# AlexeyAB/yolo2_light

Measured on NVIDIA H100. Metric: images/sec, higher is better.
Workload: dtype bf16

## Files before the change

yolo2_light_b200/csrc/yb_conv_tc.cu:

```cuda
#include <cuda.h>
#include <cuda_bf16.h>
#include <cuda_runtime.h>

#include <algorithm>
#include <climits>
#include <cstdlib>
#include <cstring>
#include <string>
#include <type_traits>
#include <vector>

#include "yb_conv_tc.cuh"

namespace yb {

namespace {

constexpr int TC_BM = 128;
constexpr int TC_EPI_WARPS = 8;
constexpr int TC_THREADS = 32 * TC_EPI_WARPS + 32;
constexpr int TC_PRODUCER_WARP = TC_EPI_WARPS;
constexpr int TC_ACC_BAR = 3;

struct TcParams {
// ... 765 lines not shown
                const int img = J / p.PR, oy = J - img * p.PR - p.row_off;
                valid[h] = img < p.N && oy >= 0 && oy < p.OH && ox < p.OW;
            }
            const int nslab = (min(BN, p.n - n0) + SW - 1) / SW;
            if constexpr (ST) {
                const long long c0 = clock64();
                mbar_wait(stg_ready(wg), stg_phase);
                const long long dt = clock64() - c0;
                if (w != w_first) w_ready += dt;
                else if (p.stats && warp == 0 && lane == 0) p.stats[blockIdx.x * 16 + 3] = (unsigned long long)dt;
            }
            else mbar_wait(stg_ready(wg), stg_phase);
            stg_phase ^= 1u;
#pragma unroll
            for (int s = 0; s < BN / SW; ++s) {
                if (s >= nslab) break;
                const uint32_t slab = buf + (uint32_t)s * TILE;
#pragma unroll
                for (int jj = 0; jj < SW / 8; ++jj) {
                    const int j = s * (SW / 8) + jj;
                    const float2 b = *reinterpret_cast<const float2 *>(bias_s + n0 + 8 * j + cq);
#pragma unroll
                    for (int e = 0; e < 4; ++e) {
                        const float a = d[4 * j + e] + ((e & 1) ? b.y : b.x);
                        d[4 * j + e] = leaky ? fmaxf(a, 0.1f * a) : a;
                    }
                }
                if (has_res) {
                    uint32_t u[SW / 8][2];
#pragma unroll
                    for (int jj = 0; jj < SW / 8; ++jj)
#pragma unroll
                        for (int h = 0; h < 2; ++h)
                            asm volatile("ld.shared.b32 %0, [%1];" : "=r"(u[jj][h]) : "r"(slab + slab_off(rl + 8 * h, jj)));
#pragma unroll
                    for (int jj = 0; jj < SW / 8; ++jj) {
                        const int j = s * (SW / 8) + jj;
#pragma unroll
                        for (int h = 0; h < 2; ++h) {
                            float a = d[4 * j + 2 * h] + __uint_as_float(u[jj][h] << 16);
                            float c = d[4 * j + 2 * h + 1] + __uint_as_float(u[jj][h] & 0xffff0000u);
                            if (leaky2) { a = fmaxf(a, 0.1f * a); c = fmaxf(c, 0.1f * c); }
                            d[4 * j + 2 * h] = a; d[4 * j + 2 * h + 1] = c;
                        }
                    }
                }
#pragma unroll
                for (int jj = 0; jj < SW / 8; ++jj) {
                    const int j = s * (SW / 8) + jj;
#pragma unroll
                    for (int h = 0; h < 2; ++h) {
                        const uint32_t o = valid[h] ? pack_bf16x2(d[4 * j + 2 * h], d[4 * j + 2 * h + 1]) : 0u;
                        asm volatile("st.shared.b32 [%0], %1;" ::"r"(slab + slab_off(rl + 8 * h, jj)), "r"(o));
                    }
                }
                asm volatile("fence.proxy.async.shared::cta;" ::: "memory");
                __syncwarp();
                if (lane == 0) mbar_arrive(stg_full(wg, s));
            }
        }
    };
    auto by_kk = [&](auto bn_c) {
        if (p.kk == 4) run(bn_c, std::integral_constant<int, 4>{});
        else if (p.kk == 2) run(bn_c, std::integral_constant<int, 2>{});
        else run(bn_c, std::integral_constant<int, 1>{});
    };
    if (p.BN == 256) by_kk(std::integral_constant<int, 256>{});
    else if (p.BN == 128) by_kk(std::integral_constant<int, 128>{});
    else if (p.BN == 64) by_kk(std::integral_constant<int, 64>{});
    else by_kk(std::integral_constant<int, 32>{});
    if (ST && p.stats && warp == 0 && lane == 0) { p.stats[blockIdx.x * 16 + 2] = (unsigned long long)w_full; p.stats[blockIdx.x * 16 + 6] = (unsigned long long)(clock64() - t_begin);
                                                    p.stats[blockIdx.x * 16 + 8] = (unsigned long long)w_ready; }
}

struct StemTcP {
    const float *in;
    const unsigned char *in8;
    char *out; int out_ldc;
    const __nv_bfloat16 *w;
    const float *bias;
    int N, H, W, OHp, OWp, nf, act;
    long npix;
    int ntiles;
};

template <bool U8>
__global__ void __launch_bounds__(128) k_stem_tc(StemTcP p) {
    __shared__ __align__(1024) uint8_t a_tile[128 * 64];
    __shared__ __align__(1024) uint8_t b_tile[32 * 64];
    __shared__ __align__(16) float acc_s[128 * 36];
    __shared__ float bias_s[32];
    __shared__ unsigned long long optr[128];
    __shared__ float lut[U8 ? 256 : 1];
    const int t = threadIdx.x;
    if constexpr (U8) { lut[t] = (float)((double)(float)t / 255.0); lut[t + 128] = (float)((double)(float)(t + 128) / 255.0); }
    const uint32_t a_addr = smem_u32(a_tile), b_addr = smem_u32(b_tile), acc_addr = smem_u32(acc_s);
    if (t < 32) bias_s[t] = (t < p.nf) ? p.bias[t] : 0.f;
    {
        const int f = t >> 2, j = t & 3;
        const uint4 v = *reinterpret_cast<const uint4 *>(p.w + f * 32 + j * 8);
        *reinterpret_cast<uint4 *>(b_tile + f * 64 + ((j ^ ((f >> 1) & 3)) << 4)) = v;
    }
    __syncthreads();
    const uint32_t hi = ((8u * 64u) >> 4) | (2u << 30);
    const size_t plane = (size_t)p.H * p.W;
    for (int tile = blockIdx.x; tile < p.ntiles; tile += gridDim.x) {
        const unsigned pix = (unsigned)tile * 128u + (unsigned)t;
        const bool ok = pix < (unsigned)p.npix;
        int x = 0, y = 0, n = 0;
        if (ok) { const unsigned row = pix / (unsigned)p.W; x = (int)(pix - row * (unsigned)p.W); n = (int)(row / (unsigned)p.H); y = (int)(row - (unsigned)n * (unsigned)p.H); }
        uint32_t packed[16];
        {
            float v[32];
            if constexpr (U8) {
                const unsigned char *img8 = p.in8 + (size_t)n * 3 * plane;
                if (ok && x >= 1 && x + 1 < p.W && y >= 1 && y + 1 < p.H) {
                    const unsigned char *r1 = img8 + ((size_t)y * p.W + x) * 3, *r0 = r1 - (size_t)p.W * 3, *r2 = r1 + (size_t)p.W * 3;
#pragma unroll
                    for (int j = 0; j < 9; ++j) {
                        v[0 * 9 + j] = lut[__ldg(r0 - 3 + j)];
                        v[1 * 9 + j] = lut[__ldg(r1 - 3 + j)];
                        v[2 * 9 + j] = lut[__ldg(r2 - 3 + j)];
                    }
                } else {
#pragma unroll
                    for (int ky = 0; ky < 3; ++ky)
#pragma unroll
                        for (int kx = 0; kx < 3; ++kx) {
                            const int iy = y + ky - 1, ix = x + kx - 1;
                            const bool in_img = ok && iy >= 0 && iy < p.H && ix >= 0 && ix < p.W;
#pragma unroll
                            for (int c = 0; c < 3; ++c)
                                v[(ky * 3 + kx) * 3 + c] = in_img ? lut[__ldg(img8 + ((size_t)iy * p.W + ix) * 3 + c)] : 0.f;
                        }
                }
            } else {
            const float *img = p.in + (size_t)n * 3 * plane;
            if (ok && x >= 1 && x + 1 < p.W && y >= 1 && y + 1 < p.H) {
                const float *c0 = img + (size_t)y * p.W + x;
#pragma unroll
                for (int c = 0; c < 3; ++c) {
                    const float *r1 = c0 + (size_t)c * plane, *r0 = r1 - p.W, *r2 = r1 + p.W;
                    v[(0 * 3 + 0) * 3 + c] = __ldg(r0 - 1); v[(0 * 3 + 1) * 3 + c] = __ldg(r0); v[(0 * 3 + 2) * 3 + c] = __ldg(r0 + 1);
                    v[(1 * 3 + 0) * 3 + c] = __ldg(r1 - 1); v[(1 * 3 + 1) * 3 + c] = __ldg(r1); v[(1 * 3 + 2) * 3 + c] = __ldg(r1 + 1);
                    v[(2 * 3 + 0) * 3 + c] = __ldg(r2 - 1); v[(2 * 3 + 1) * 3 + c] = __ldg(r2); v[(2 * 3 + 2) * 3 + c] = __ldg(r2 + 1);
                }
            } else {
#pragma unroll
            for (int ky = 0; ky < 3; ++ky)
#pragma unroll
                for (int kx = 0; kx < 3; ++kx) {
                    const int iy = y + ky - 1, ix = x + kx - 1;
                    const bool in_img = ok && iy >= 0 && iy < p.H && ix >= 0 && ix < p.W;
#pragma unroll
                    for (int c = 0; c < 3; ++c)
                        v[(ky * 3 + kx) * 3 + c] = in_img ? __ldg(img + (size_t)c * plane + (size_t)iy * p.W + ix) : 0.f;
                }
            }
            }
#pragma unroll
            for (int k = 27; k < 32; ++k) v[k] = 0.f;
#pragma unroll
            for (int k = 0; k < 16; ++k) packed[k] = pack_bf16x2(v[2 * k], v[2 * k + 1]);
        }
#pragma unroll
        for (int j = 0; j < 4; ++j)
            *reinterpret_cast<uint4 *>(a_tile + t * 64 + ((j ^ ((t >> 1) & 3)) << 4)) =
                make_uint4(packed[4 * j], packed[4 * j + 1], packed[4 * j + 2], packed[4 * j + 3]);
        asm volatile("fence.proxy.async.shared::cta;" ::: "memory");
        __syncthreads();
        {
            float d0[16], d1[16];
#pragma unroll
            for (int i = 0; i < 16; ++i) { d0[i] = 0.f; d1[i] = 0.f; }
            wg_fence();
#pragma unroll
            for (int k = 0; k < 2; ++k) {
                const uint64_t bdesc = wg_desc(b_addr + 32u * k, hi);
                Wg<0, 32>::mma(d0, wg_desc(a_addr + 32u * k, hi), bdesc, (uint32_t)k);
                Wg<0, 32>::mma(d1, wg_desc(a_addr + 64u * 64u + 32u * k, hi), bdesc, (uint32_t)k);
            }
            wg_commit();
            wg_wait<0>();
            acc_store_frag(acc_addr, 36, 0, d0);
            acc_store_frag(acc_addr, 36, 64, d1);
        }
        __syncthreads();
        uint32_t acc[32];
        acc_ld32(acc_addr + 4u * 36u * (uint32_t)t, acc);
        char *orow = ok ? p.out + ((size_t)(n * p.OHp + y + 1) * p.OWp + x + 1) * (size_t)p.out_ldc * 2 : nullptr;
        if (p.nf == 32) {
            uint4 o[4];
#pragma unroll
            for (int g = 0; g < 4; ++g) {
                float r[8];
#pragma unroll
                for (int j = 0; j < 8; ++j) {
                    const float a = __uint_as_float(acc[g * 8 + j]) + bias_s[g * 8 + j];
                    r[j] = (p.act == ACT_LEAKY) ? fmaxf(a, 0.1f * a) : a;
                }
                o[g] = make_uint4(pack_bf16x2(r[0], r[1]), pack_bf16x2(r[2], r[3]), pack_bf16x2(r[4], r[5]), pack_bf16x2(r[6], r[7]));
            }
#pragma unroll
            for (int g = 0; g < 4; ++g) *reinterpret_cast<uint4 *>(a_tile + t * 64 + ((g ^ ((t >> 1) & 3)) << 4)) = o[g];
            optr[t] = (unsigned long long)(uintptr_t)orow;
            __syncthreads();
#pragma unroll
            for (int k = 0; k < 4; ++k) {
                const int j = t + 128 * k, px = j >> 2, part = j & 3;
                const unsigned long long dst = optr[px];
                if (dst)
                    *reinterpret_cast<uint4 *>(dst + (unsigned long long)(part * 16)) =
                        *reinterpret_cast<const uint4 *>(a_tile + px * 64 + ((part ^ ((px >> 1) & 3)) << 4));
            }
        } else if (ok) {
#pragma unroll
            for (int g = 0; g < 4; ++g) {
                if (g * 8 >= p.nf) break;
                float r[8];
#pragma unroll
                for (int j = 0; j < 8; ++j) {
                    const float a = __uint_as_float(acc[g * 8 + j]) + bias_s[g * 8 + j];
                    r[j] = (p.act == ACT_LEAKY) ? fmaxf(a, 0.1f * a) : a;
                }
                reinterpret_cast<uint4 *>(orow)[g] = make_uint4(pack_bf16x2(r[0], r[1]), pack_bf16x2(r[2], r[3]),
                                                                pack_bf16x2(r[4], r[5]), pack_bf16x2(r[6], r[7]));
            }
        }
        __syncthreads();
    }
}

typedef CUresult (*EncodeTiledFn)(CUtensorMap *, CUtensorMapDataType, cuuint32_t, void *, const cuuint64_t *,
                                  const cuuint64_t *, const cuuint32_t *, const cuuint32_t *, CUtensorMapInterleave,
                                  CUtensorMapSwizzle, CUtensorMapL2promotion, CUtensorMapFloatOOBfill);

EncodeTiledFn encode_fn() {
    static EncodeTiledFn fn = nullptr;
    if (!fn) {
        void *p = nullptr;
        cudaDriverEntryPointQueryResult q;
        if (cudaGetDriverEntryPoint("cuTensorMapEncodeTiled", &p, cudaEnableDefault, &q) != cudaSuccess || !p)
            fatal_throw("cuTensorMapEncodeTiled not available from the driver");
        fn = reinterpret_cast<EncodeTiledFn>(p);
    }
    return fn;
}

struct TcPlan {
    CUtensorMap tmA, tmB, tmO, tmO1, tmR;
    TcParams p;
    int grid;
    int threads;
    size_t smem;
    int pdl;
    char desc[96];
};

int pick_bk(int C) { return (C % 64 == 0) ? 64 : (C % 32 == 0) ? 32 : (C % 16 == 0) ? 16 : 0; }
int pick_bk_i8(int cpad) { return (cpad % 128 == 0) ? 128 : (cpad % 64 == 0) ? 64 : (cpad % 32 == 0) ? 32 : 0; }
int pick_bk_f32(int C) { return (C % 32 == 0) ? 32 : (C % 16 == 0) ? 16 : (C % 8 == 0) ? 8 : 0; }
int pick_bn(int n) { return n <= 32 ? 32 : n <= 64 ? 64 : 128; }
int pick_bn_reg(int n, long m_tiles, int kblocks, int sms) {
    int cap = 32;
    while (cap < n && cap < 256) cap *= 2;
    if (const char *e = getenv("YB_TC_BN")) {
        int bn = 32;
        while (bn * 2 <= std::min(atoi(e), cap)) bn *= 2;
        return bn;
    }
    int best = 32; double best_cost = 1e300;
    for (int bn = 32; bn <= cap; bn *= 2) {
        const long items = m_tiles * ((n + bn - 1) / bn);
        const double cost = (double)((items + sms - 1) / sms) * ((double)kblocks * (bn + 64) + 2.0 * bn);
        if (cost < best_cost) { best_cost = cost; best = bn; }
    }
    return best;
}

int grid_cap(int sms) {
    const char *e = getenv("YB_TC_GRID");
    return (e && atoi(e) > 0) ? std::min(sms, atoi(e)) : sms;
}

}

int tc_conv_supported(const Layer &l, const TV &in, const TV &out, bool out_bf16) {
    if (!out.base || (reinterpret_cast<uintptr_t>(out.base) & 15) != 0) return 0;
    if (out_bf16 ? (out.ldc % 8 != 0) : (out.ldc % 4 != 0)) return 0;
    if (l.activation != YB_LEAKY && l.activation != YB_LINEAR) return 0;
    if (pick_bk(l.c) == 0) return 0;
    if (in.ldc % 8 != 0 || (reinterpret_cast<uintptr_t>(in.base) & 15) != 0 || in.P != 1) return 0;
    const bool s1 = l.stride == 1 && ((l.size == 3 && l.pad == 1) || (l.size == 1 && l.pad == 0));
    const bool s2 = l.stride == 2 && l.size == 3 && l.pad == 1 && (l.h % 2 == 0) && (l.w % 2 == 0);
    if (!s1 && !s2) return 0;
    if (out_bf16 && l.n % 8 != 0) return 0;
    if (l.n < 8) return 0;
    return 1;
}

static void *make_plan_common(int kind, const Layer &l, const TV &in, const TV &out, bool out_bf16, const TV &res,
                              bool res_bf16, int act2, const void *d_weights_bf16, int ldn, const float *d_bias,
                              float alpha1, int *acc_out, int wide_rows = 0, int want_pool_tile = 0) {
    TcPlan *plan = new TcPlan();
    memset(plan, 0, sizeof(*plan));
    TcParams &p = plan->p;
    const bool i8 = kind == 1 || kind == 2;
    const int esz = kind == 3 ? 4 : i8 ? 1 : 2;
    const int cin = i8 ? in.ldc : l.c;
    const int BK = kind == 3 ? pick_bk_f32(l.c) : i8 ? pick_bk_i8(cin) : pick_bk(l.c);
    const bool reg = kind == 0 && out_bf16;
    p.kind = kind; p.alpha1 = alpha1; p.acc_out = acc_out;
// ... 141 lines not shown
    plan->threads = reg ? TCR_THREADS : TC_THREADS;
    if (getenv("YB_TC_STATS")) {
        cudaMalloc(&p.stats, sizeof(unsigned long long) * 16 * plan->grid);
        cudaMemset(p.stats, 0, sizeof(unsigned long long) * 16 * plan->grid);
    }
    plan->smem = 1024  + p.bstat_bytes + (size_t)p.stages * p.stage_bytes + 8 * (2 * p.stages + 11) + 16 +
                 sizeof(float) * (size_t)p.nt * BN  + (size_t)p.nt * BN / 8  +
                 (p.tma_epi ? 1024 : 128) + p.stg_bytes  +
                 acc_bytes ;
    if (plan->smem > 227 * 1024) { delete plan; fatal_throw("tc plan: shared memory budget exceeded"); }
    {
        const void *fns[] = {(const void *)k_conv_tc<false, 0>, (const void *)k_conv_tc_reg<false>, (const void *)k_conv_tc<false, 2>,
                             (const void *)k_conv_tc<true, 0>, (const void *)k_conv_tc_reg<true>, (const void *)k_conv_tc<true, 2>};
        for (const void *f : fns)
            if (cudaFuncSetAttribute(f, cudaFuncAttributeMaxDynamicSharedMemorySize, 227 * 1024) != cudaSuccess)
                fatal_throw("cudaFuncSetAttribute(k_conv_tc) failed");
    }
    return plan;
}

void *tc_make_plan(const Layer &l, const TV &in, const TV &out, bool out_bf16, const TV &res, bool res_bf16,
                   int act2, const void *d_weights_bf16, int ldn, const float *d_bias, int wide_rows) {
    return make_plan_common(0, l, in, out, out_bf16, res, res_bf16, act2, d_weights_bf16, ldn, d_bias, 0.f, nullptr, wide_rows);
}

int tc_tf32_supported(const Layer &l, const TV &in, const TV &out) {
    if (pick_bk_f32(l.c) == 0) return 0;
    if ((reinterpret_cast<uintptr_t>(in.base) & 15) != 0 || in.P != 1 || in.ldc % 4 != 0) return 0;
    const bool s1 = l.stride == 1 && ((l.size == 3 && l.pad == 1) || (l.size == 1 && l.pad == 0));
    const bool s2 = l.stride == 2 && l.size == 3 && l.pad == 1 && (l.h % 2 == 0) && (l.w % 2 == 0);
    if (!s1 && !s2) return 0;
    if (!out.base || (reinterpret_cast<uintptr_t>(out.base) & 15) != 0 || out.ldc % 4 != 0 || l.n < 8) return 0;
    if (l.activation != YB_LEAKY && l.activation != YB_LINEAR) return 0;
    return 1;
}
void *tc_make_plan_tf32(const Layer &l, const TV &in, const TV &out, const void *d_weights_f32, int ldn, const float *d_bias,
                        int wide_rows) {
    TV none{};
    return make_plan_common(3, l, in, out, false, none, false, ACT_LINEAR, d_weights_f32, ldn, d_bias, 0.f, nullptr, wide_rows);
}

int tc_i8_supported(const Layer &l, const TV &q, const TV &out) {
    if (pick_bk_i8(q.ldc) == 0) return 0;
    if ((reinterpret_cast<uintptr_t>(q.base) & 15) != 0 || q.P != 1 || q.ldc % 16 != 0) return 0;
    const bool s1 = l.stride == 1 && ((l.size == 3 && l.pad == 1) || (l.size == 1 && l.pad == 0));
    const bool s2 = l.stride == 2 && l.size == 3 && l.pad == 1 && (l.h % 2 == 0) && (l.w % 2 == 0);
    if (!s1 && !s2) return 0;
    if (!out.base || (reinterpret_cast<uintptr_t>(out.base) & 15) != 0 || out.ldc % 4 != 0 || l.n < 8) return 0;
    if (l.activation != YB_LEAKY && l.activation != YB_LINEAR) return 0;
    return 1;
}
void tc_plan_fuse_yolo(void *vp, float *d_yolo_nchw, int classes) {
    TcPlan *plan = reinterpret_cast<TcPlan *>(vp);
    plan->p.yolo_out = d_yolo_nchw;
    plan->p.yolo_per = 4 + classes + 1;
}

int tc_plan_fuse_pool(void *vp, int mode, float mult, const TV &qnext) {
    TcPlan *plan = reinterpret_cast<TcPlan *>(vp);
    TcParams &p = plan->p;
    if (!(p.kind == 1 || p.kind == 2) || p.TW != 8 || p.jshift != 1 || (p.PR & 1) || (p.OW & 1) || (p.OH & 1) || p.acc_out) return 0;
    if (qnext.H != p.OH / 2 || qnext.W != p.OW / 2 || qnext.ldc % 16 != 0 || (reinterpret_cast<uintptr_t>(qnext.base) & 15) || p.n % 32 != 0) return 0;
    p.pool_mode = mode; p.pool_mult = mult;
    p.pool_out = reinterpret_cast<signed char *>(qnext.base); p.pool_ldc = qnext.ldc; p.pool_Hp = qnext.Hp; p.pool_Wp = qnext.Wp;
    return 1;
}

void *tc_make_plan_i8(const Layer &l, const TV &q, const TV &out, const void *d_weights_s8, int ldn, const float *d_bias,
                      float alpha1, int *acc_out, int want_pool_tile) {
    TV none{};
    return make_plan_common(1, l, q, out, false, none, false, ACT_LINEAR, d_weights_s8, ldn, d_bias, alpha1, acc_out, 0, want_pool_tile);
}

void *tc_make_plan_xnor(const Layer &l, const TV &q, const TV &out, const void *d_weights_pm1, int ldn, const float *d_bias,
                        const float *d_mean, int *counts_out, int want_pool_tile) {
    TV none{};
    TcPlan *plan = reinterpret_cast<TcPlan *>(
        make_plan_common(2, l, q, out, false, none, false, ACT_LINEAR, d_weights_pm1, ldn, d_bias, 0.f, counts_out, 0, want_pool_tile));
    plan->p.mean = d_mean;
    plan->p.xK = l.size * l.size * l.c;
    return plan;
}

struct StemPlan { StemTcP p; int grid; };
int tc_stem_supported(const Layer &l, const TV &out) {
    return l.c == 3 && l.size == 3 && l.stride == 1 && l.pad == 1 && (l.n == 16 || l.n == 32) &&
           (l.activation == YB_LEAKY || l.activation == YB_LINEAR) && out.base && out.ldc % 8 == 0 &&
           (reinterpret_cast<uintptr_t>(out.base) & 15) == 0;
}
void *tc_stem_make_plan(const Layer &l, const TV &out, const void *d_w, const float *d_bias) {
    StemPlan *sp = new StemPlan();
    memset(sp, 0, sizeof(*sp));
    StemTcP &p = sp->p;
    p.out = out.base; p.out_ldc = out.ldc; p.w = reinterpret_cast<const __nv_bfloat16 *>(d_w); p.bias = d_bias;
    p.N = out.N; p.H = l.h; p.W = l.w; p.OHp = out.Hp; p.OWp = out.Wp; p.nf = l.n; p.act = l.activation;
    p.npix = (long)out.N * l.h * l.w;
    if (p.npix >= (1L << 31) - 256) fatal_throw("stem plan: more than 2^31 pixels per batch");
    p.ntiles = (int)((p.npix + 127) / 128);
    int dev = 0, sms = 132;
    cudaGetDevice(&dev);
    cudaDeviceGetAttribute(&sms, cudaDevAttrMultiProcessorCount, dev);
    sp->grid = std::min(p.ntiles, sms * 8);
    return sp;
}
void tc_stem_launch(void *vp, const float *d_in_nchw, cudaStream_t s) {
    StemPlan *sp = reinterpret_cast<StemPlan *>(vp);
    StemTcP p = sp->p;
    p.in = d_in_nchw;
    k_stem_tc<false><<<sp->grid, 128, 0, s>>>(p);
}
void tc_stem_launch_u8(void *vp, const unsigned char *d_in_hwc, cudaStream_t s) {
    StemPlan *sp = reinterpret_cast<StemPlan *>(vp);
    StemTcP p = sp->p;
    p.in8 = d_in_hwc;
    k_stem_tc<true><<<sp->grid, 128, 0, s>>>(p);
}
void tc_stem_free_plan(void *vp) { delete reinterpret_cast<StemPlan *>(vp); }

void tc_launch(void *vp, cudaStream_t s) {
    TcPlan *plan = reinterpret_cast<TcPlan *>(vp);
    cudaLaunchConfig_t cfg{};
    cfg.gridDim = dim3((unsigned)plan->grid); cfg.blockDim = dim3((unsigned)plan->threads);
    cfg.dynamicSmemBytes = plan->smem; cfg.stream = s;
    cudaLaunchAttribute attr[2];
    int na = 0;
    if (plan->pdl) {
        attr[na].id = cudaLaunchAttributeProgrammaticStreamSerialization;
        attr[na].val.programmaticStreamSerializationAllowed = 1;
        ++na;
    }
    cfg.attrs = attr; cfg.numAttrs = na;
    const bool st = plan->p.stats != nullptr;
    const TcPlan &P = *plan;
#define YB_TC_LAUNCH(KERNEL) cudaLaunchKernelEx(&cfg, KERNEL, P.tmA, P.tmB, P.tmO, P.tmR, P.p)
    if (plan->threads == TCR_THREADS) {
        if (st) cudaLaunchKernelEx(&cfg, k_conv_tc_reg<true>, P.tmA, P.tmB, P.tmO, P.tmO1, P.tmR, P.p);
        else cudaLaunchKernelEx(&cfg, k_conv_tc_reg<false>, P.tmA, P.tmB, P.tmO, P.tmO1, P.tmR, P.p);
    }
    else if (P.p.kind == 1 || P.p.kind == 2) { if (st) YB_TC_LAUNCH((k_conv_tc<true, 2>)); else YB_TC_LAUNCH((k_conv_tc<false, 2>)); }
    else { if (st) YB_TC_LAUNCH((k_conv_tc<true, 0>)); else YB_TC_LAUNCH((k_conv_tc<false, 0>)); }
#undef YB_TC_LAUNCH
}

void tc_free_plan(void *vp) {
    TcPlan *plan = reinterpret_cast<TcPlan *>(vp);
    if (plan && plan->p.stats) {
        std::vector<unsigned long long> h(16 * (size_t)plan->grid);
        cudaDeviceSynchronize();
        cudaMemcpy(h.data(), plan->p.stats, h.size() * sizeof(unsigned long long), cudaMemcpyDeviceToHost);
        double m[16] = {0};
        for (int b = 0; b < plan->grid; ++b) for (int k = 0; k < 16; ++k) m[k] += (double)h[16 * b + k] / plan->grid;
        fprintf(stderr, "TCSTATS %-28s tiles/cta %.1f kb %d sps %d BN %d | producer: wait_empty %.0f tma_issue %.0f total %.0f | ",
                plan->desc, (double)plan->p.num_work / plan->grid, plan->p.kblocks, plan->p.sps, plan->p.BN, m[0], m[7], m[1]);
        if (plan->threads == TCR_THREADS)
            fprintf(stderr, "consumers: wait_full %.0f wait_ready %.0f (first item %.0f) total %.0f | store: wait_full %.0f wait_read %.0f\n",
                    m[2], m[8], m[3], m[6], m[4], m[5]);
        else fprintf(stderr, "consumers: wait_full %.0f wait_res %.0f total %.0f\n", m[2], m[8], m[6]);
        cudaFree(plan->p.stats);
    }
    delete plan;
}

}
```

yolo2_light_b200/csrc/yb_conv_tc.cuh:

```cuda
#pragma once
#include <cuda_runtime.h>

#include "yb_kernels.cuh"
#include "yb_model.h"

namespace yb {

int tc_conv_supported(const Layer &l, const TV &in, const TV &out, bool out_bf16);
void *tc_make_plan(const Layer &l, const TV &in, const TV &out, bool out_bf16, const TV &res, bool res_bf16,
                   int act2, const void *d_weights_bf16, int ldn, const float *d_bias, int wide_rows = 0);
int tc_tf32_supported(const Layer &l, const TV &in, const TV &out);
void *tc_make_plan_tf32(const Layer &l, const TV &in, const TV &out, const void *d_weights_f32, int ldn, const float *d_bias,
                        int wide_rows);
int tc_i8_supported(const Layer &l, const TV &q, const TV &out);
void *tc_make_plan_i8(const Layer &l, const TV &q, const TV &out, const void *d_weights_s8, int ldn, const float *d_bias,
                      float alpha1, int *acc_out, int want_pool_tile = 0);
void *tc_make_plan_xnor(const Layer &l, const TV &q, const TV &out, const void *d_weights_pm1, int ldn, const float *d_bias,
                        const float *d_mean, int *counts_out, int want_pool_tile = 0);
int tc_plan_fuse_pool(void *plan, int mode, float mult, const TV &qnext);
void tc_plan_fuse_yolo(void *plan, float *d_yolo_nchw, int classes);
int tc_stem_supported(const Layer &l, const TV &out);
void *tc_stem_make_plan(const Layer &l, const TV &out, const void *d_w_32x32_bf16, const float *d_bias);
void tc_stem_launch(void *plan, const float *d_in_nchw, cudaStream_t s);
void tc_stem_launch_u8(void *plan, const unsigned char *d_in_hwc, cudaStream_t s);
void tc_stem_free_plan(void *plan);
void tc_launch(void *plan, cudaStream_t s);
void tc_free_plan(void *plan);

}
```

yolo2_light_b200/csrc/yb_engine.cu:

```cuda
#include "yb_engine.h"

#include <cuda_bf16.h>
#include <cuda_runtime.h>
#include <dlfcn.h>

#include <algorithm>
#include <cmath>
#include <cstdlib>
#include <cstring>

#include "yb_conv_tc.cuh"
#include "yb_kernels.cuh"
#include "yb_detect.cuh"

namespace yb {

#define CUDA_OK(call)                                                                                   \
    do {                                                                                                \
        cudaError_t _e = (call);                                                                        \
        if (_e != cudaSuccess)                                                                          \
            fatal_throw(std::string("CUDA error: ") + cudaGetErrorString(_e) + " at " + __FILE__ + ":" + \
                        std::to_string(__LINE__) + " (" #call ")");                                     \
    } while (0)

// ... 405 lines not shown
                w.ldn = (int)align_up(l.n, 64);
                w.w_bf16 = reserve(sizeof(__nv_bfloat16) * (size_t)w.ldn * K);
                __nv_bfloat16 *dst = reinterpret_cast<__nv_bfloat16 *>(&hostw[w.w_bf16]);
                for (int f = 0; f < l.n; ++f)
                    for (int c = 0; c < l.c; ++c)
                        for (int t = 0; t < taps; ++t)
                            dst[(size_t)f * K + (size_t)t * l.c + c] =
                                __float2bfloat16_rn(l.weights[((size_t)f * l.c + c) * taps + t]);
            } else {
                w.ldw = (int)align_up(l.n, 64);
                w.w_f32 = reserve(sizeof(float) * (size_t)K * w.ldw);
                float *dst = reinterpret_cast<float *>(&hostw[w.w_f32]);
                for (int f = 0; f < l.n; ++f)
                    for (int c = 0; c < l.c; ++c)
                        for (int t = 0; t < taps; ++t)
                            dst[(ADT == DT_F32 ? (size_t)c * taps + t : (size_t)t * l.c + c) * w.ldw + f] =
                                l.weights[((size_t)f * l.c + c) * taps + t];
            }
        } else if (v == 1 && xnor_fallback(l)) {
            w.ldw = (int)align_up(l.n, 64);
            w.w_f32 = reserve(sizeof(float) * (size_t)K * w.ldw);
            float *dst = reinterpret_cast<float *>(&hostw[w.w_f32]);
            for (int f = 0; f < l.n; ++f)
                for (int c = 0; c < l.c; ++c)
                    for (int t = 0; t < taps; ++t)
                        dst[((size_t)c * taps + t) * w.ldw + f] = l.weights[((size_t)f * l.c + c) * taps + t] > 0 ? l.mean_arr[f] : -l.mean_arr[f];
        } else if (v == 1 && xnor_on_tc(l)) {
            w.cpad = side_ld[i];
            w.ldn = (int)align_up(l.n, 64);
            w.w_s8 = reserve((size_t)w.ldn * taps * w.cpad);
            int8_t *dst = reinterpret_cast<int8_t *>(&hostw[w.w_s8]);
            for (int f = 0; f < l.n; ++f)
                for (int c = 0; c < l.c; ++c)
                    for (int t = 0; t < taps; ++t)
                        dst[((size_t)f * taps + t) * w.cpad + c] = l.weights[((size_t)f * l.c + c) * taps + t] > 0 ? 1 : -1;
            w.mean = reserve(sizeof(float) * align_up(l.n, 64));
            memcpy(&hostw[w.mean], l.mean_arr.data(), sizeof(float) * l.n);
        } else if (v == 1) {
            const int CW = (l.c + 31) / 32;
            w.ldn = (int)align_up(l.n, 64);
            w.cpad = CW * 32;
            w.w_bits = reserve(sizeof(uint32_t) * (size_t)w.ldn * taps * CW);
            uint32_t *dst = reinterpret_cast<uint32_t *>(&hostw[w.w_bits]);
            for (int f = 0; f < l.n; ++f)
                for (int c = 0; c < l.c; ++c)
                    for (int t = 0; t < taps; ++t)
                        if (l.weights[((size_t)f * l.c + c) * taps + t] > 0)
                            dst[((size_t)f * taps + t) * CW + c / 32] |= 1u << (c & 31);
            w.mean = reserve(sizeof(float) * align_up(l.n, 64));
            memcpy(&hostw[w.mean], l.mean_arr.data(), sizeof(float) * l.n);
        } else {
            w.cpad = side_ld[i];
            w.ldn = (int)align_up(l.n, 64);
            w.w_s8 = reserve((size_t)w.ldn * taps * w.cpad);
            int8_t *dst = reinterpret_cast<int8_t *>(&hostw[w.w_s8]);
            for (int f = 0; f < l.n; ++f)
                for (int c = 0; c < l.c; ++c)
                    for (int t = 0; t < taps; ++t)
                        dst[((size_t)f * taps + t) * w.cpad + c] = l.weights_int8[((size_t)f * l.c + c) * taps + t];
        }
    }
    size_t stem_w_off = (size_t)-1;
    {
        const Layer &l0 = net->layers[0];
        if (ADT == DT_BF16 && l0.type == YB_CONVOLUTIONAL && conv_variant(0) == 0 && l0.c == 3 && l0.size == 3 && l0.n <= 32) {
            stem_w_off = reserve(sizeof(__nv_bfloat16) * 32 * 32);
            __nv_bfloat16 *dst = reinterpret_cast<__nv_bfloat16 *>(&hostw[stem_w_off]);
            for (int i = 0; i < 32 * 32; ++i) dst[i] = __float2bfloat16_rn(0.f);
            for (int f = 0; f < l0.n; ++f)
                for (int c = 0; c < 3; ++c)
                    for (int t = 0; t < 9; ++t)
                        dst[f * 32 + t * 3 + c] = __float2bfloat16_rn(l0.weights[((size_t)f * 3 + c) * 9 + t]);
        }
    }
    e->w_bytes = align_up(std::max<size_t>(hostw.size(), 1024), 1024);
    CUDA_OK(cudaMalloc(&e->w_arena, e->w_bytes));
    if (opt.upload) CUDA_OK(cudaMemcpyAsync(e->w_arena, hostw.data(), hostw.size(), cudaMemcpyHostToDevice, e->stream));
    CUDA_OK(cudaStreamSynchronize(e->stream));

    e->input_count = (size_t)B * net->c * net->h * net->w;
    CUDA_OK(cudaMalloc(&e->d_input, e->input_count * sizeof(float)));

    Engine *E = e.get();
    bool stem_fused = false, stem_pool_fused = false;
    {
        const Layer &l0 = net->layers[0];
        const bool stem_ok = l0.type == YB_CONVOLUTIONAL && conv_variant(0) == 0 && !use_tc[0] && l0.c == 3 &&
                             l0.size == 3 && l0.stride == 1 && l0.pad == 1 && (l0.n == 16 || l0.n == 32) &&
                             fused_into[0] < 0 && e->out_tv[0].base && !getenv("YB_NO_STEM") &&
                             (e->out_dt[0] == DT_F32 || (e->out_tv[0].ldc % 8 == 0));
        bool pool_ok = stem_ok && opt.fuse && e->out_dt[0] == DT_F32 && l0.n == 16 && nl > 2 && !getenv("YB_NO_STEM_POOL_FUSE") &&
                       (l0.activation == YB_LEAKY || l0.activation == YB_LINEAR);
        if (pool_ok) {
            const Layer &mp = net->layers[1], &c2 = net->layers[2];
            pool_ok = mp.type == YB_MAXPOOL && mp.size == 2 && mp.stride == 2 && mp.pad == 1 && cons[0].size() == 1 && cons[0][0] == 1 &&
                      cons[1].size() == 1 && cons[1][0] == 2 && c2.type == YB_CONVOLUTIONAL && conv_variant(2) != 0 &&
                      side_off[2] != (size_t)-1 && !xnor_fallback(c2) && (conv_variant(2) == 1 && !xnor_on_tc(c2) ? true : side_ld[2] % 16 == 0);
        }
        if (pool_ok) {
            stem_fused = true; stem_pool_fused = true;
            const Layer &c2 = net->layers[2];
            const int v2 = conv_variant(2);
            const bool pm1 = v2 == 1 && xnor_on_tc(c2);
            const TV q = (v2 == 2 || pm1) ? make_tv(e->act_arena + side_off[2], B, c2.h, c2.w, c2.c, side_ld[2], P, DT_S8, 0)
                                          : make_tv(e->act_arena + side_off[2], B, c2.h, c2.w, side_ld[2], side_ld[2], P, DT_BITS, 0);
            StemW<16> w16{};
            for (int f = 0; f < 16; ++f) {
                for (int c = 0; c < 3; ++c)
                    for (int t = 0; t < 9; ++t) w16.w[(t * 3 + c) * 16 + f] = l0.weights[((size_t)f * 3 + c) * 9 + t];
                w16.b[f] = l0.biases[f];
            }
            const int act = l0.activation, H = l0.h, W = l0.w;
            const float mult = (v2 == 2) ? c2.input_quant_multipler : 0.f;
            const int grid = (int)(((long)B * c2.h * c2.w + 127) / 128);
            prefilled[2] = 1;
            e->not_materialised[0] = e->not_materialised[1] = 1;
            e->first_kind = OP_CONV_SIMT; e->first_layer = 0;
            e->first_op = [=](const float *din, cudaStream_t s) {
                if (v2 == 2 && act == ACT_LEAKY) k_stem_pool<0, ACT_LEAKY><<<grid, 128, 0, s>>>(din, q, w16, act, H, W, mult);
                else if (v2 == 2) k_stem_pool<0, ACT_LINEAR><<<grid, 128, 0, s>>>(din, q, w16, act, H, W, mult);
                else if (pm1 && act == ACT_LEAKY) k_stem_pool<1, ACT_LEAKY><<<grid, 128, 0, s>>>(din, q, w16, act, H, W, mult);
                else if (pm1) k_stem_pool<1, ACT_LINEAR><<<grid, 128, 0, s>>>(din, q, w16, act, H, W, mult);
                else if (act == ACT_LEAKY) k_stem_pool<2, ACT_LEAKY><<<grid, 128, 0, s>>>(din, q, w16, act, H, W, mult);
                else k_stem_pool<2, ACT_LINEAR><<<grid, 128, 0, s>>>(din, q, w16, act, H, W, mult);
            };
        } else if (stem_ok && stem_w_off != (size_t)-1 && e->out_dt[0] == DT_BF16 && tc_stem_supported(l0, e->out_tv[0]) &&
            !getenv("YB_NO_STEM_TC")) {
            stem_fused = true;
            void *sp = tc_stem_make_plan(l0, e->out_tv[0], e->w_arena + stem_w_off,
                                         reinterpret_cast<const float *>(e->w_arena + cw[0].bias));
            e->stem_plan = sp;
            e->first_kind = OP_CONV_TC; e->first_layer = 0;
            e->first_op = [sp](const float *din, cudaStream_t s) { tc_stem_launch(sp, din, s); };
            if (!getenv("YB_NO_STEM_U8")) e->first_op_u8 = [sp](const unsigned char *d8, cudaStream_t s) { tc_stem_launch_u8(sp, d8, s); };
        } else if (stem_ok) {
            stem_fused = true;
            const TV tout = e->out_tv[0];
            const int act = l0.activation, H = l0.h, W = l0.w, nf = l0.n, odt = e->out_dt[0];
            StemW<32> w32{}; StemW<16> w16{};
            for (int f = 0; f < nf; ++f) {
                for (int c = 0; c < 3; ++c)
                    for (int t = 0; t < 9; ++t) {
                        const float v = l0.weights[((size_t)f * 3 + c) * 9 + t];
                        if (nf == 32) w32.w[(t * 3 + c) * 32 + f] = v; else w16.w[(t * 3 + c) * 16 + f] = v;
                    }
                if (nf == 32) w32.b[f] = l0.biases[f]; else w16.b[f] = l0.biases[f];
            }
            const long total = (long)B * H * W;
            const int grid = (int)((total + 127) / 128);
            e->first_kind = OP_CONV_SIMT; e->first_layer = 0;
            e->first_op = [=](const float *din, cudaStream_t s) {
                if (nf == 32 && odt == DT_BF16) k_conv_stem<32, __nv_bfloat16><<<grid, 128, 0, s>>>(din, tout, w32, act, H, W);
                else if (nf == 32) k_conv_stem<32, float, true><<<grid, 128, 0, s>>>(din, tout, w32, act, H, W);
                else if (odt == DT_BF16) k_conv_stem<16, __nv_bfloat16><<<grid, 128, 0, s>>>(din, tout, w16, act, H, W);
                else k_conv_stem<16, float, true><<<grid, 128, 0, s>>>(din, tout, w16, act, H, W);
            };
        } else {
            const TV in0 = e->in0;
            const int dt = e->in0_dt;
            const int g = grid_for((long)in0.N * in0.H * in0.W);
            e->first_op = [=](const float *din, cudaStream_t s) {
                if (dt == DT_F32) k_input_nchw_to_nhwc<float><<<g, 256, 0, s>>>(din, in0);
                else k_input_nchw_to_nhwc<__nv_bfloat16><<<g, 256, 0, s>>>(din, in0);
            };
        }
        e->ops.push_back(Op{e->first_kind, e->first_layer, nullptr});
    }
    for (int i = 0; i < nl; ++i) {
        const Layer &l = net->layers[i];
        const TV tin = (i == 0) ? e->in0 : e->out_tv[i - 1];
        const int in_dt = (i == 0) ? e->in0_dt : e->out_dt[i - 1];
        const bool prev_ok = (i == 0) || e->out_tv[i - 1].base != nullptr;
        auto need_prev = [&]() {
            if (!prev_ok) fatal_throw("engine: layer " + std::to_string(i) + " has no image input");
        };
        if (i == 0 && stem_fused) continue;
        if (i == 1 && stem_pool_fused) continue;
        switch (l.type) {
        case YB_CONVOLUTIONAL: {
            need_prev();
            const int v = conv_variant(i);
            const int tgt = fused_into[i] >= 0 ? fused_into[i] : i;
            const TV tout = e->out_tv[tgt];
            const int odt = e->out_dt[tgt];
            if (!tout.base) fatal_throw("engine: conv output not placed");
            if (tin.C != l.c || tin.H != l.h || tin.W != l.w) fatal_throw("engine: conv input shape mismatch");
            const long M = (long)B * l.out_h * l.out_w;
            if (v == 0) {
                TV res{}; int rdt = DT_F32; int act2 = ACT_LINEAR;
                if (fused_into[i] >= 0) {
                    const Layer &s = net->layers[tgt];
                    res = e->out_tv[s.index];
                    rdt = e->out_dt[s.index];
                    act2 = s.activation;
                    if (!res.base) fatal_throw("engine: shortcut source not placed");
                }
                if (use_tc[i] == 2) {
                    const bool fuse_yolo = opt.fuse && i + 1 < nl && net->layers[i + 1].type == YB_YOLO && cons[i].size() == 1 &&
                                           cons[i][0] == i + 1 && e->d_final[i + 1] && !getenv("YB_NO_YOLO_FUSE");
                    void *plan = tc_make_plan_tf32(l, tin, tout, e->w_arena + cw[i].w_f32km, cw[i].ldn,
                                                   reinterpret_cast<const float *>(e->w_arena + cw[i].bias), fuse_yolo ? 1 : 0);
                    e->tc_plans.push_back(plan);
                    ++e->n_tc;
                    if (fuse_yolo) {
                        tc_plan_fuse_yolo(plan, e->d_final[i + 1], net->layers[i + 1].classes);
                        yolo_fused[i + 1] = 1;
                    }
                    e->ops.push_back(Op{OP_CONV_TC_TF32, i, [plan](cudaStream_t s) { tc_launch(plan, s); }});
                } else if (use_tc[i]) {
                    const bool fuse_yolo = opt.fuse && fused_into[i] < 0 && odt == DT_F32 && i + 1 < nl &&
                                           net->layers[i + 1].type == YB_YOLO && cons[i].size() == 1 && cons[i][0] == i + 1 &&
                                           e->d_final[i + 1] && !getenv("YB_NO_YOLO_FUSE");
                    void *plan = tc_make_plan(l, tin, tout, odt == DT_BF16, res, rdt == DT_BF16, act2,
                                              e->w_arena + cw[i].w_bf16, cw[i].ldn,
                                              reinterpret_cast<const float *>(e->w_arena + cw[i].bias), fuse_yolo ? 1 : 0);
                    e->tc_plans.push_back(plan);
                    ++e->n_tc;
                    if (fuse_yolo) {
                        tc_plan_fuse_yolo(plan, e->d_final[i + 1], net->layers[i + 1].classes);
                        yolo_fused[i + 1] = 1;
                    }
                    e->ops.push_back(Op{OP_CONV_TC, i, [plan](cudaStream_t s) { tc_launch(plan, s); }});
                } else {
                    ConvP p{};
                    p.in = tin; p.out = tout; p.res = res;
                    p.w = e->w_arena + cw[i].w_f32;
                    p.bias = reinterpret_cast<const float *>(e->w_arena + cw[i].bias);
                    p.n = l.n; p.ldw = cw[i].ldw; p.size = l.size; p.stride = l.stride; p.pad = l.pad;
                    p.act = l.activation; p.act2 = act2; p.K = l.size * l.size * l.c; p.M = M;
                    dim3 grid((unsigned)((M + 63) / 64), (unsigned)((l.n + 63) / 64));
                    const int key = in_dt * 4 + odt * 2 + rdt;
                    e->ops.push_back(Op{OP_CONV_SIMT, i, [p, grid, key](cudaStream_t s) {
                        switch (key) {
                        case 0: k_conv_simt<float, float, float, true><<<grid, 256, 0, s>>>(p); break;
                        case 1: k_conv_simt<float, float, __nv_bfloat16><<<grid, 256, 0, s>>>(p); break;
                        case 2: k_conv_simt<float, __nv_bfloat16, float><<<grid, 256, 0, s>>>(p); break;
                        case 3: k_conv_simt<float, __nv_bfloat16, __nv_bfloat16><<<grid, 256, 0, s>>>(p); break;
                        case 4: k_conv_simt<__nv_bfloat16, float, float><<<grid, 256, 0, s>>>(p); break;
                        case 5: k_conv_simt<__nv_bfloat16, float, __nv_bfloat16><<<grid, 256, 0, s>>>(p); break;
                        case 6: k_conv_simt<__nv_bfloat16, __nv_bfloat16, float><<<grid, 256, 0, s>>>(p); break;
                        default: k_conv_simt<__nv_bfloat16, __nv_bfloat16, __nv_bfloat16><<<grid, 256, 0, s>>>(p); break;
                        }
                    }});
                }
            } else if (v == 1) {
                if (in_dt != DT_F32 || odt != DT_F32) fatal_throw("engine: xnor path needs f32 activations");
                if (xnor_fallback(l)) {
                    TV pm1 = make_tv(e->act_arena + side_off[i], B, l.h, l.w, l.c, l.c, P, DT_F32, 0);
                    const int gb = grid_for((long)B * l.h * l.w * l.c);
                    e->ops.push_back(Op{OP_BINARIZE, i, [tin, pm1, gb](cudaStream_t s) { k_binarize_pm1<<<gb, 256, 0, s>>>(tin, pm1); }});
                    ConvP p{};
                    p.in = pm1; p.out = tout; p.res = TV{};
                    p.w = e->w_arena + cw[i].w_f32;
                    p.bias = reinterpret_cast<const float *>(e->w_arena + cw[i].bias);
                    p.n = l.n; p.ldw = cw[i].ldw; p.size = l.size; p.stride = l.stride; p.pad = l.pad;
                    p.act = l.activation; p.act2 = ACT_LINEAR; p.K = l.size * l.size * l.c; p.M = M;
                    dim3 grid((unsigned)((M + 63) / 64), (unsigned)((l.n + 63) / 64));
                    e->ops.push_back(Op{OP_CONV_SIMT, i, [p, grid](cudaStream_t s) { k_conv_simt<float, float, float, true><<<grid, 256, 0, s>>>(p); }});
                    break;
                }
// ... 760 lines not shown
```

Measured before the change: 2489.

## Fuse stem conv with following stride-2 conv in one tensor-core kernel

Adds a persistent kernel that computes the 3-channel stem convolution into shared memory for a tile with halo, then immediately runs the stride-2 3x3 conv (32->64) with wgmma from shared memory, writing only the second layer's output. This avoids materialising the full-resolution 32-channel stem activation in global memory and a separate launch for layer 1. It adds halo recomputation, large dynamic shared memory and a software-prefetched input patch, and is enabled only when the network shapes match.

```diff
diff --git a/yolo2_light_b200/csrc/yb_conv_tc.cu b/yolo2_light_b200/csrc/yb_conv_tc.cu
--- a/yolo2_light_b200/csrc/yb_conv_tc.cu
+++ b/yolo2_light_b200/csrc/yb_conv_tc.cu
@@ -871,6 +871,9 @@
     int N, H, W, OHp, OWp, nf, act;
     long npix;
     int ntiles;
+    const __nv_bfloat16 *w1;
+    const float *bias1;
+    int act1, OH, OW, xt, yt;
 };
 
 template <bool U8>
@@ -1017,6 +1020,210 @@
             }
         }
         __syncthreads();
+    }
+}
+
+constexpr int S2_TW = 16, S2_TH = 8;
+constexpr int S2_RW = 2 * S2_TW + 1, S2_RH = 2 * S2_TH + 1;
+constexpr int S2_ROWS = 640;
+constexpr uint32_t S2_B1 = 0;
+constexpr uint32_t S2_BS = 9u * 4096u;
+constexpr uint32_t S2_U = S2_BS + 2048u;
+constexpr uint32_t S2_SETS_KX = 17u * 1024u;
+constexpr uint32_t S2_STG = (uint32_t)S2_ROWS * 64u;
+constexpr uint32_t S2_MISC = S2_U + S2_STG + 2u * 8192u;
+constexpr int S2_PH = S2_RH + 2, S2_PW = S2_RW + 2, S2_PP = 36;
+constexpr size_t S2_SMEM = 1024 + S2_MISC + 4 * (32 + 64 + 256) + 4 * 3 * S2_PH * S2_PP;
+static_assert(S2_STG + 2u * 8192u >= 3u * S2_SETS_KX, "sets must fit the shared region");
+
+template <bool U8>
+__global__ void __launch_bounds__(256, 2) k_stem_s2_tc(StemTcP p) {
+    extern __shared__ uint8_t smem_raw[];
+    uint8_t *sm = smem_raw + ((1024u - (smem_u32(smem_raw) & 1023u)) & 1023u);
+    const uint32_t base = smem_u32(sm), U = base + S2_U;
+    float *bias0_s = reinterpret_cast<float *>(sm + S2_MISC), *bias1_s = bias0_s + 32, *lut = bias1_s + 64, *patch = lut + 256;
+    const int t = threadIdx.x, lane = t & 31;
+    const int warp = __shfl_sync(0xffffffffu, t >> 5, 0), wg = warp >> 2;
+    if constexpr (U8) lut[t] = (float)((double)(float)t / 255.0);
+    if (t < 32) bias0_s[t] = p.bias[t];
+    if (t < 64) bias1_s[t] = p.bias1[t];
+    if (t < 128) {
+        const int f = t >> 2, j = t & 3;
+        *reinterpret_cast<uint4 *>(sm + S2_BS + f * 64 + ((j ^ ((f >> 1) & 3)) << 4)) = *reinterpret_cast<const uint4 *>(p.w + f * 32 + j * 8);
+    }
+    for (int i = t; i < 9 * 64 * 4; i += 256) {
+        const int r = i >> 8, f = (i >> 2) & 63, j = i & 3;
+        *reinterpret_cast<uint4 *>(sm + S2_B1 + r * 4096 + f * 64 + ((j ^ ((f >> 1) & 3)) << 4)) =
+            *reinterpret_cast<const uint4 *>(p.w1 + f * 288 + r * 32 + j * 8);
+    }
+    asm volatile("fence.proxy.async.shared::cta;" ::: "memory");
+    __syncthreads();
+
+    const uint32_t hi = ((8u * 64u) >> 4) | (2u << 30);
+    const bool leaky0 = p.act == ACT_LEAKY, leaky1 = p.act1 == ACT_LEAKY;
+    const int rl = 16 * (warp & 3) + (lane >> 2), cq = 2 * (lane & 3);
+    constexpr int PER = (3 * S2_PH * S2_PW + 255) / 256;
+    auto patch_index = [&](int e, int &c, int &r, int &col) {
+        if constexpr (U8) { r = e / (3 * S2_PW); const int b = e - r * 3 * S2_PW; col = b / 3; c = b - col * 3; }
+        else { c = e / (S2_PH * S2_PW); const int b = e - c * S2_PH * S2_PW; r = b / S2_PW; col = b - r * S2_PW; }
+    };
+    auto load_patch = [&](int tile, float (&v)[PER]) {
+        const int tx = tile % p.xt, rest = tile / p.xt, ty = rest % p.yt, n = rest / p.yt;
+        const int py0 = 2 * ty * S2_TH - 2, px0 = 2 * tx * S2_TW - 2;
+        const size_t img = (size_t)n * 3 * p.H * p.W;
+#pragma unroll
+        for (int k = 0; k < PER; ++k) {
+            const int e = t + 256 * k;
+            int c, r, col;
+            patch_index(e, c, r, col);
+            const int y = py0 + r, x = px0 + col;
+            const bool in_img = e < 3 * S2_PH * S2_PW && y >= 0 && y < p.H && x >= 0 && x < p.W;
+            if constexpr (U8) v[k] = in_img ? lut[__ldg(p.in8 + img + (unsigned)((y * p.W + x) * 3 + c))] : 0.f;
+            else v[k] = in_img ? __ldg(p.in + img + (unsigned)((c * p.H + y) * p.W + x)) : 0.f;
+        }
+    };
+    float pv[PER];
+    if ((int)blockIdx.x < p.ntiles) load_patch(blockIdx.x, pv);
+    for (int tile = blockIdx.x; tile < p.ntiles; tile += gridDim.x) {
+        const int tx = tile % p.xt, rest = tile / p.xt, ty = rest % p.yt, n = rest / p.yt;
+        const int ox0 = tx * S2_TW, oy0 = ty * S2_TH;
+        const int gy0 = 2 * oy0 - 1, gx0 = 2 * ox0 - 1;
+
+#pragma unroll
+        for (int k = 0; k < PER; ++k) {
+            const int e = t + 256 * k;
+            if (e >= 3 * S2_PH * S2_PW) break;
+            int c, r, col;
+            patch_index(e, c, r, col);
+            patch[(c * S2_PH + r) * S2_PP + col] = pv[k];
+        }
+        __syncthreads();
+
+        for (int i = t; i < S2_ROWS; i += 256) {
+            const int sy = i / S2_RW, sx = i - sy * S2_RW;
+            const float *w0 = patch + sy * S2_PP + sx;
+            const bool ok = i < S2_RW * S2_RH;
+            uint32_t packed[16];
+            {
+                float v[32];
+#pragma unroll
+                for (int ky = 0; ky < 3; ++ky)
+#pragma unroll
+                    for (int kx = 0; kx < 3; ++kx)
+#pragma unroll
+                        for (int c = 0; c < 3; ++c) v[(ky * 3 + kx) * 3 + c] = ok ? w0[(c * S2_PH + ky) * S2_PP + kx] : 0.f;
+#pragma unroll
+                for (int k = 27; k < 32; ++k) v[k] = 0.f;
+#pragma unroll
+                for (int k = 0; k < 16; ++k) packed[k] = pack_bf16x2(v[2 * k], v[2 * k + 1]);
+            }
+#pragma unroll
+            for (int j = 0; j < 4; ++j)
+                *reinterpret_cast<uint4 *>(sm + S2_U + i * 64 + ((j ^ ((i >> 1) & 3)) << 4)) =
+                    make_uint4(packed[4 * j], packed[4 * j + 1], packed[4 * j + 2], packed[4 * j + 3]);
+        }
+        asm volatile("fence.proxy.async.shared::cta;" ::: "memory");
+        __syncthreads();
+
+        float ds[5][16];
+#pragma unroll
+        for (int c = 0; c < 5; ++c)
+#pragma unroll
+            for (int i = 0; i < 16; ++i) ds[c][i] = 0.f;
+#pragma unroll
+        for (int c = 0; c < 5; ++c) wg_fence_operand(ds[c]);
+        wg_fence();
+#pragma unroll
+        for (int c = 0; c < 5; ++c)
+#pragma unroll
+            for (int k = 0; k < 2; ++k)
+                Wg<0, 32>::mma(ds[c], wg_desc(U + (uint32_t)(5 * wg + c) * 4096u + 32u * k, hi), wg_desc(base + S2_BS + 32u * k, hi), (uint32_t)k);
+        wg_commit();
+        wg_wait<0>();
+#pragma unroll
+        for (int c = 0; c < 5; ++c) wg_fence_operand(ds[c]);
+        __syncthreads();
+
+        {
+#pragma unroll
+            for (int c = 0; c < 5; ++c)
+#pragma unroll
+                for (int h = 0; h < 2; ++h) {
+                    const int i = 64 * (5 * wg + c) + rl + 8 * h;
+                    if (i >= S2_RW * S2_RH) continue;
+                    const int sy = i / S2_RW, sx = i - sy * S2_RW, y = gy0 + sy, x = gx0 + sx;
+                    const bool in_img = y >= 0 && y < p.H && x >= 0 && x < p.W;
+                    uint32_t v[4];
+#pragma unroll
+                    for (int j = 0; j < 4; ++j) {
+                        float a = ds[c][4 * j + 2 * h] + bias0_s[8 * j + cq], b = ds[c][4 * j + 2 * h + 1] + bias0_s[8 * j + cq + 1];
+                        if (leaky0) { a = fmaxf(a, 0.1f * a); b = fmaxf(b, 0.1f * b); }
+                        v[j] = in_img ? pack_bf16x2(a, b) : 0u;
+                    }
+                    const uint32_t set = U + ((sy & 1) ? 9u * 1024u : 0u) + (uint32_t)(sy >> 1) * 1024u + 2u * (uint32_t)cq;
+                    auto put = [&](int kx, int ox) {
+                        const uint32_t row = set + (uint32_t)kx * S2_SETS_KX + (uint32_t)ox * 64u;
+#pragma unroll
+                        for (int j = 0; j < 4; ++j)
+                            asm volatile("st.shared.b32 [%0], %1;" ::"r"(row + ((uint32_t)(j ^ ((ox >> 1) & 3)) << 4)), "r"(v[j]));
+                    };
+                    const bool odd = sx & 1, last = sx == 2 * S2_TW;
+                    put(odd ? 1 : last ? 2 : 0, last ? (sx >> 1) - 1 : sx >> 1);
+                    if (!odd && !last && sx >= 2) put(2, (sx >> 1) - 1);
+                }
+        }
+        asm volatile("fence.proxy.async.shared::cta;" ::: "memory");
+        __syncthreads();
+
+        if (tile + (int)gridDim.x < p.ntiles) load_patch(tile + gridDim.x, pv);
+
+        float d[32];
+#pragma unroll
+        for (int i = 0; i < 32; ++i) d[i] = 0.f;
+        wg_fence_operand(d);
+        wg_fence();
+#pragma unroll
+        for (int r = 0; r < 9; ++r) {
+            const int ky = r / 3, kx = r % 3;
+            const uint32_t a = U + (uint32_t)kx * S2_SETS_KX + ((ky & 1) ? 9u * 1024u : 0u) + (uint32_t)(ky >> 1) * 1024u + (uint32_t)wg * 4096u;
+            const uint32_t b = base + S2_B1 + (uint32_t)r * 4096u;
+#pragma unroll
+            for (int k = 0; k < 2; ++k)
+                Wg<0, 64>::mma(d, wg_desc(a + 32u * k, hi), wg_desc(b + 32u * k, hi), (r > 0 || k > 0) ? 1u : 0u);
+        }
+        wg_commit();
+        wg_wait<0>();
+        wg_fence_operand(d);
+        __syncthreads();
+
+        const uint32_t stg = U + S2_STG + (uint32_t)wg * 8192u;
+        float b1[16];
+#pragma unroll
+        for (int j = 0; j < 8; ++j) { b1[2 * j] = bias1_s[8 * j + cq]; b1[2 * j + 1] = bias1_s[8 * j + cq + 1]; }
+#pragma unroll
+        for (int h = 0; h < 2; ++h) {
+            const int q = rl + 8 * h;
+#pragma unroll
+            for (int j = 0; j < 8; ++j) {
+                float a = d[4 * j + 2 * h] + b1[2 * j], b = d[4 * j + 2 * h + 1] + b1[2 * j + 1];
+                if (leaky1) { a = fmaxf(a, 0.1f * a); b = fmaxf(b, 0.1f * b); }
+                asm volatile("st.shared.b32 [%0], %1;" ::"r"(stg + (uint32_t)q * 128u + ((uint32_t)(j ^ (q & 7)) << 4) + 2u * (uint32_t)cq),
+                             "r"(pack_bf16x2(a, b)) : "memory");
+            }
+        }
+        if (wg == 0) named_bar_sync(1, 128);
+        else named_bar_sync(2, 128);
+#pragma unroll
+        for (int k = 0; k < 4; ++k) {
+            const int idx = (t & 127) + 128 * k, q = idx >> 3, ch = idx & 7;
+            const int oy = oy0 + 4 * wg + (q >> 4), ox = ox0 + (q & 15);
+            if (oy < p.OH && ox < p.OW) {
+                uint4 o;
+                asm volatile("ld.shared.v4.b32 {%0, %1, %2, %3}, [%4];" : "=r"(o.x), "=r"(o.y), "=r"(o.z), "=r"(o.w)
+                             : "r"(stg + (uint32_t)q * 128u + ((uint32_t)(ch ^ (q & 7)) << 4)) : "memory");
+                *reinterpret_cast<uint4 *>(p.out + ((size_t)(n * p.OHp + oy + 1) * p.OWp + ox + 1) * (size_t)p.out_ldc * 2 + ch * 16) = o;
+            }
+        }
     }
 }
 
@@ -1324,7 +1531,7 @@
     return plan;
 }
 
-struct StemPlan { StemTcP p; int grid; };
+struct StemPlan { StemTcP p; int grid; bool s2; };
 int tc_stem_supported(const Layer &l, const TV &out) {
     return l.c == 3 && l.size == 3 && l.stride == 1 && l.pad == 1 && (l.n == 16 || l.n == 32) &&
            (l.activation == YB_LEAKY || l.activation == YB_LINEAR) && out.base && out.ldc % 8 == 0 &&
@@ -1345,17 +1552,49 @@
     sp->grid = std::min(p.ntiles, sms * 8);
     return sp;
 }
+int tc_stem_s2_supported(const Layer &l0, const Layer &l1, const TV &out1) {
+    return l0.n == 32 && l1.c == 32 && l1.n == 64 && l1.size == 3 && l1.stride == 2 && l1.pad == 1 && l1.h == l0.h && l1.w == l0.w &&
+           l0.h % 2 == 0 && l0.w % 2 == 0 && (l1.activation == YB_LEAKY || l1.activation == YB_LINEAR) && out1.base && out1.P == 1 &&
+           out1.H == l0.h / 2 && out1.W == l0.w / 2 && out1.ldc % 8 == 0 && (reinterpret_cast<uintptr_t>(out1.base) & 15) == 0;
+}
+void *tc_stem_s2_make_plan(const Layer &l0, const Layer &l1, const TV &out1, const void *d_w, const float *d_bias, const void *d_w1,
+                           const float *d_bias1) {
+    StemPlan *sp = new StemPlan();
+    memset(sp, 0, sizeof(*sp));
+    sp->s2 = true;
+    StemTcP &p = sp->p;
+    p.out = out1.base; p.out_ldc = out1.ldc; p.w = reinterpret_cast<const __nv_bfloat16 *>(d_w); p.bias = d_bias;
+    p.N = out1.N; p.H = l0.h; p.W = l0.w; p.OHp = out1.Hp; p.OWp = out1.Wp; p.nf = l0.n; p.act = l0.activation;
+    p.w1 = reinterpret_cast<const __nv_bfloat16 *>(d_w1); p.bias1 = d_bias1; p.act1 = l1.activation;
+    p.OH = out1.H; p.OW = out1.W;
+    p.xt = (p.OW + S2_TW - 1) / S2_TW; p.yt = (p.OH + S2_TH - 1) / S2_TH;
+    const long ntiles = (long)p.N * p.xt * p.yt;
+    if (ntiles >= INT_MAX) fatal_throw("stem plan: too many tiles");
+    p.ntiles = (int)ntiles;
+    int dev = 0, sms = 132;
+    cudaGetDevice(&dev);
+    cudaDeviceGetAttribute(&sms, cudaDevAttrMultiProcessorCount, dev);
+    sp->grid = std::min(p.ntiles, grid_cap(2 * sms));
+    for (const void *f : {(const void *)k_stem_s2_tc<false>, (const void *)k_stem_s2_tc<true>}) {
+        if (cudaFuncSetAttribute(f, cudaFuncAttributeMaxDynamicSharedMemorySize, (int)S2_SMEM) != cudaSuccess ||
+            cudaFuncSetAttribute(f, cudaFuncAttributePreferredSharedMemoryCarveout, 100) != cudaSuccess)
+            fatal_throw("cudaFuncSetAttribute(k_stem_s2_tc) failed");
+    }
+    return sp;
+}
 void tc_stem_launch(void *vp, const float *d_in_nchw, cudaStream_t s) {
     StemPlan *sp = reinterpret_cast<StemPlan *>(vp);
     StemTcP p = sp->p;
     p.in = d_in_nchw;
-    k_stem_tc<false><<<sp->grid, 128, 0, s>>>(p);
+    if (sp->s2) k_stem_s2_tc<false><<<sp->grid, 256, S2_SMEM, s>>>(p);
+    else k_stem_tc<false><<<sp->grid, 128, 0, s>>>(p);
 }
 void tc_stem_launch_u8(void *vp, const unsigned char *d_in_hwc, cudaStream_t s) {
     StemPlan *sp = reinterpret_cast<StemPlan *>(vp);
     StemTcP p = sp->p;
     p.in8 = d_in_hwc;
-    k_stem_tc<true><<<sp->grid, 128, 0, s>>>(p);
+    if (sp->s2) k_stem_s2_tc<true><<<sp->grid, 256, S2_SMEM, s>>>(p);
+    else k_stem_tc<true><<<sp->grid, 128, 0, s>>>(p);
 }
 void tc_stem_free_plan(void *vp) { delete reinterpret_cast<StemPlan *>(vp); }
 
diff --git a/yolo2_light_b200/csrc/yb_conv_tc.cuh b/yolo2_light_b200/csrc/yb_conv_tc.cuh
--- a/yolo2_light_b200/csrc/yb_conv_tc.cuh
+++ b/yolo2_light_b200/csrc/yb_conv_tc.cuh
@@ -21,6 +21,9 @@
 void tc_plan_fuse_yolo(void *plan, float *d_yolo_nchw, int classes);
 int tc_stem_supported(const Layer &l, const TV &out);
 void *tc_stem_make_plan(const Layer &l, const TV &out, const void *d_w_32x32_bf16, const float *d_bias);
+int tc_stem_s2_supported(const Layer &l0, const Layer &l1, const TV &out1);
+void *tc_stem_s2_make_plan(const Layer &l0, const Layer &l1, const TV &out1, const void *d_w_32x32_bf16, const float *d_bias,
+                           const void *d_w1_bf16, const float *d_bias1);
 void tc_stem_launch(void *plan, const float *d_in_nchw, cudaStream_t s);
 void tc_stem_launch_u8(void *plan, const unsigned char *d_in_hwc, cudaStream_t s);
 void tc_stem_free_plan(void *plan);
diff --git a/yolo2_light_b200/csrc/yb_engine.cu b/yolo2_light_b200/csrc/yb_engine.cu
--- a/yolo2_light_b200/csrc/yb_engine.cu
+++ b/yolo2_light_b200/csrc/yb_engine.cu
@@ -511,7 +511,7 @@
     CUDA_OK(cudaMalloc(&e->d_input, e->input_count * sizeof(float)));
 
     Engine *E = e.get();
-    bool stem_fused = false, stem_pool_fused = false;
+    bool stem_fused = false, stem_pool_fused = false, stem_s2_fused = false;
     {
         const Layer &l0 = net->layers[0];
         const bool stem_ok = l0.type == YB_CONVOLUTIONAL && conv_variant(0) == 0 && !use_tc[0] && l0.c == 3 &&
@@ -556,10 +556,20 @@
         } else if (stem_ok && stem_w_off != (size_t)-1 && e->out_dt[0] == DT_BF16 && tc_stem_supported(l0, e->out_tv[0]) &&
             !getenv("YB_NO_STEM_TC")) {
             stem_fused = true;
-            void *sp = tc_stem_make_plan(l0, e->out_tv[0], e->w_arena + stem_w_off,
-                                         reinterpret_cast<const float *>(e->w_arena + cw[0].bias));
+            const float *bias0 = reinterpret_cast<const float *>(e->w_arena + cw[0].bias);
+            stem_s2_fused = opt.fuse && !getenv("YB_NO_STEM_S2_FUSE") && nl > 1 && cons[0].size() == 1 && cons[0][0] == 1 &&
+                            net->layers[1].type == YB_CONVOLUTIONAL && conv_variant(1) == 0 && use_tc[1] == 1 &&
+                            fused_into[1] < 0 && e->out_dt[1] == DT_BF16 && tc_stem_s2_supported(l0, net->layers[1], e->out_tv[1]);
+            void *sp = stem_s2_fused ? tc_stem_s2_make_plan(l0, net->layers[1], e->out_tv[1], e->w_arena + stem_w_off, bias0,
+                                                            e->w_arena + cw[1].w_bf16, reinterpret_cast<const float *>(e->w_arena + cw[1].bias))
+                                     : tc_stem_make_plan(l0, e->out_tv[0], e->w_arena + stem_w_off, bias0);
             e->stem_plan = sp;
             e->first_kind = OP_CONV_TC; e->first_layer = 0;
+            if (stem_s2_fused) {
+                e->not_materialised[0] = 1;
+                e->first_layer = 1;
+                ++e->n_tc;
+            }
             e->first_op = [sp](const float *din, cudaStream_t s) { tc_stem_launch(sp, din, s); };
             if (!getenv("YB_NO_STEM_U8")) e->first_op_u8 = [sp](const unsigned char *d8, cudaStream_t s) { tc_stem_launch_u8(sp, d8, s); };
         } else if (stem_ok) {
@@ -604,7 +614,7 @@
             if (!prev_ok) fatal_throw("engine: layer " + std::to_string(i) + " has no image input");
         };
         if (i == 0 && stem_fused) continue;
-        if (i == 1 && stem_pool_fused) continue;
+        if (i == 1 && (stem_pool_fused || stem_s2_fused)) continue;
         switch (l.type) {
         case YB_CONVOLUTIONAL: {
             need_prev();
```

Result: faster. 2580 (median of 6 runs) (+3.7%).
